# yahoo/bftkv

Hardware: AMD Instinct MI355X
Metric: pgp_rsa2048_signature_verifies_per_sec (higher is better)
Workload: dtype u32; 1 GPU; 64-replica quorum, 10000 RSA-2048 signed writes per GPU (cfg2 of BASELINE.json), 534164 signature packets per GPU, 1.0% corrupt / 0.5% unknown issuer / 0.5% duplicate / 1.0% one-short; parallelism=shard-by-write x1, RCCL all-gather of verdict bitmaps on the verifier's stream, replicas=64, writes_per_gpu=10000, sigs_per_gpu=534164, batches_in_flight=3

## Files before the change

### bftkv_amd/csrc/mont28.h

```cpp
#pragma once
#include <hip/hip_runtime.h>
#include <stdint.h>

namespace bftkv {

constexpr int MONT_W = 28;
constexpr uint32_t MONT_MASK = (1u << MONT_W) - 1;
constexpr int MONT_TPI = 4;
constexpr int MONT_L = 19;
constexpr int MONT_N = MONT_TPI * MONT_L;
constexpr int MONT_TPI_BIG = 8;
constexpr int MONT_L3072 = 14, MONT_L4096 = 19;
constexpr int MONT_NMAX = MONT_TPI_BIG * MONT_L4096;

constexpr int DPP_QUAD_BCAST0 = 0x00;
constexpr int DPP_QUAD_SHR1 = 0x90;
constexpr int DPP_QUAD_SWAP1 = 0xB1;
constexpr int DPP_QUAD_SWAP2 = 0x4E;
constexpr int DPP_ROW_SHL1 = 0x101;

__device__ __forceinline__ uint32_t dpp_quad_bcast0(uint32_t v) {
  return (uint32_t)__builtin_amdgcn_update_dpp(0, (int)v, DPP_QUAD_BCAST0, 0xF, 0xF, true);
}
__device__ __forceinline__ uint32_t dpp_quad_shr1(uint32_t v) {
  return (uint32_t)__builtin_amdgcn_update_dpp(0, (int)v, DPP_QUAD_SHR1, 0xF, 0xF, false);
}
__device__ __forceinline__ uint32_t dpp_row_shl1(uint32_t v) {
  return (uint32_t)__builtin_amdgcn_update_dpp(0, (int)v, DPP_ROW_SHL1, 0xF, 0xF, true);
}
constexpr int DPP_ROW_SHR1 = 0x111;
constexpr int DPP_ROW_SHR4 = 0x114;
__device__ __forceinline__ uint32_t dpp_row_shr1(uint32_t v) {
  return (uint32_t)__builtin_amdgcn_update_dpp(0, (int)v, DPP_ROW_SHR1, 0xF, 0xF, true);
}
__device__ __forceinline__ uint32_t dpp_row_shr4(uint32_t v) {
  return (uint32_t)__builtin_amdgcn_update_dpp(0, (int)v, DPP_ROW_SHR4, 0xF, 0xF, true);
}
__device__ __forceinline__ uint32_t quad_or(uint32_t v) {
  v |= (uint32_t)__builtin_amdgcn_update_dpp(0, (int)v, DPP_QUAD_SWAP1, 0xF, 0xF, false);
  v |= (uint32_t)__builtin_amdgcn_update_dpp(0, (int)v, DPP_QUAD_SWAP2, 0xF, 0xF, false);
  return v;
}

template <int TPI>
__device__ __forceinline__ uint32_t grp_bcast0(uint32_t v, int glane) {
  const uint32_t q = dpp_quad_bcast0(v);
  if constexpr (TPI == 4) return q;
  else { const uint32_t u = dpp_row_shr4(q); return (glane & 4) ? u : q; }
}
template <int TPI>
__device__ __forceinline__ uint32_t grp_shr1(uint32_t v) {
  if constexpr (TPI == 4) return dpp_quad_shr1(v);
  else return dpp_row_shr1(v);
}
template <int TPI>
__device__ __forceinline__ uint32_t grp_or(uint32_t v) {
  v = quad_or(v);
  if constexpr (TPI == 8) v |= (uint32_t)__shfl_xor((int)v, 4);
  return v;
}

__device__ __forceinline__ uint64_t mad64(uint32_t a, uint32_t b, uint64_t c) {
  return (uint64_t)a * (uint64_t)b + c;
}

template <int L, int TPI = MONT_TPI, bool SQR = false>
__device__ __forceinline__ void mont_mul(uint32_t (&out)[L], const uint32_t* a_lds,
                                         const uint32_t (&b)[L], const uint32_t (&n)[L],
                                         uint32_t n0inv, int qlane) {
  constexpr bool NORM = 2 * TPI * L > 255;
  uint32_t mask_v;
  asm("v_mov_b32 %0, 0xfffffff" : "=v"(mask_v));
  uint64_t Q[2 * L - 1];
#pragma unroll
  for (int k = 0; k < L + (NORM ? 1 : 0); ++k) Q[k] = 0;

#pragma unroll 1
  for (int blk = 0; blk < TPI; ++blk) {
    const uint32_t* ap = a_lds + blk * L;
#pragma unroll
    for (int r = 0; r < L; ++r) {
      const uint32_t ai = ap[r];
      const uint32_t ai2 = ai << 1;
#pragma unroll
      for (int k = SQR ? r : 0; k < L; ++k) {
        const uint32_t av = (SQR && k > r) ? ai2 : ai;
        if (k == L - 1 && r > 0) Q[r + k] = mad64(av, b[k], (NORM && r == 1) ? Q[r + k] : 0);
        else Q[r + k] = mad64(av, b[k], Q[r + k]);
      }
      const uint32_t m = grp_bcast0<TPI>((uint32_t)Q[r] * n0inv, qlane) & mask_v;
#pragma unroll
      for (int k = 0; k < L; ++k) Q[r + k] = mad64(m, n[k], Q[r + k]);
      Q[r + 1] += Q[r] >> MONT_W;
    }
#pragma unroll
    for (int k = 0; k < L; ++k) {
      const uint64_t nx = dpp_row_shl1((uint32_t)Q[k]) & mask_v;
      Q[k] = (k < L - 1) ? Q[L + k] + nx : nx;
    }
    if (NORM) {
#pragma unroll
      for (int k = 0; k < L; ++k) {
        const uint64_t c = Q[k] >> MONT_W;
        Q[k] &= MONT_MASK;
        if (k < L - 1) Q[k + 1] += c; else Q[L] = c;
      }
    }
  }

  uint64_t c = 0;
#pragma unroll
  for (int k = 0; k < L; ++k) {
    uint64_t v = Q[k] + c;
    out[k] = (uint32_t)v & MONT_MASK;
    c = v >> MONT_W;
  }
  if (NORM) c += Q[L];
  uint32_t clo = grp_shr1<TPI>((uint32_t)c), chi = grp_shr1<TPI>((uint32_t)(c >> 32));
  uint64_t cin = (qlane == 0) ? 0 : (((uint64_t)chi << 32) | clo);
  uint64_t v0 = (uint64_t)out[0] + cin;
  out[0] = (uint32_t)v0 & MONT_MASK;
  uint32_t v1 = out[1] + (uint32_t)(v0 >> MONT_W);
  out[1] = v1 & MONT_MASK;
  out[2] += v1 >> MONT_W;
}

template <int L, int TPI = MONT_TPI>
__device__ __forceinline__ void canonicalize(uint32_t (&x)[L], int qlane) {
  uint32_t cout = 0;
#pragma unroll
  for (int step = 0; step < TPI; ++step) {
    uint32_t c = grp_shr1<TPI>(cout);
    if (qlane == 0) c = 0;
#pragma unroll
    for (int k = 0; k < L; ++k) {
      uint32_t v = x[k] + c;
      x[k] = v & MONT_MASK;
      c = v >> MONT_W;
    }
    cout = c;
  }
}

template <int L, int TPI = MONT_TPI>
__device__ __forceinline__ void reduce_once(uint32_t (&y)[L], const uint32_t (&n)[L], int qlane) {
  uint32_t ge = 1;
#pragma unroll
  for (int k = 0; k < L; ++k) ge = (y[k] > n[k]) ? 1u : ((y[k] < n[k]) ? 0u : ge);
  if (!__any(ge != 0 && qlane == TPI - 1)) return;
  uint32_t d[L];
#pragma unroll
  for (int k = 0; k < L; ++k) d[k] = y[k] - n[k];
  int32_t cout = 0, top = 0;
#pragma unroll
  for (int step = 0; step < TPI; ++step) {
    int32_t c = (int32_t)grp_shr1<TPI>((uint32_t)cout);
    if (qlane == 0) c = 0;
#pragma unroll
    for (int k = 0; k < L; ++k) {
      const int32_t v = (int32_t)d[k] + c;
      d[k] = (uint32_t)v & MONT_MASK;
      c = v >> MONT_W;
    }
    cout = c;
    top += c;
  }
  uint32_t keep = (top == 0) ? 1u : 0u;
  if constexpr (TPI == 4) keep = (uint32_t)__builtin_amdgcn_update_dpp(0, (int)keep, 0xFF, 0xF, 0xF, true);
  else keep = (uint32_t)__shfl((int)keep, (int)((threadIdx.x & 63u) | (uint32_t)(TPI - 1)));
  if (keep) {
#pragma unroll
    for (int k = 0; k < L; ++k) y[k] = d[k];
  }
}

}
```

Baseline: 146.8 million verifies/s.

## Use a rotating ring window for the Montgomery accumulator instead of shifting Q

In the non-normalized path (RSA-2048: L=19, TPI=4), the accumulator Q becomes a 2L-entry ring with compile-time rotating offsets, and two limb-blocks are unrolled per loop iteration. This removes the per-block copy of Q[L+k] down to Q[k]. The cross-lane DPP shift-in is folded into the next row's final multiply-add instead of a separate pass. The cost is one extra 64-bit accumulator and a doubled unrolled body, which could raise VGPR pressure and code size.

```diff
diff --git a/bftkv_amd/csrc/mont28.h b/bftkv_amd/csrc/mont28.h
--- a/bftkv_amd/csrc/mont28.h
+++ b/bftkv_amd/csrc/mont28.h
@@ -64,41 +64,72 @@
   return (uint64_t)a * (uint64_t)b + c;
 }
 
+template <int L, int TPI, bool SQR, int O>
+__device__ __forceinline__ void mont_block_ring(uint64_t (&Q)[2 * L], const uint32_t* ap, const uint32_t (&b)[L],
+                                                const uint32_t (&n)[L], uint32_t n0inv, int qlane, uint32_t mask_v) {
+  constexpr int M = 2 * L;
+#pragma unroll
+  for (int r = 0; r < L; ++r) {
+    const uint32_t ai = ap[r];
+    const uint32_t ai2 = ai << 1;
+    uint64_t in = 0;
+    if (r > 0) in = dpp_row_shl1((uint32_t)Q[(O + r - 1) % M]) & mask_v;
+#pragma unroll
+    for (int k = SQR ? r : 0; k < L; ++k) {
+      const uint32_t av = (SQR && k > r) ? ai2 : ai;
+      if (k == L - 1 && r > 0) Q[(O + r + k) % M] = mad64(av, b[k], in);
+      else Q[(O + r + k) % M] = mad64(av, b[k], Q[(O + r + k) % M]);
+    }
+    const uint32_t m = grp_bcast0<TPI>((uint32_t)Q[(O + r) % M] * n0inv, qlane) & mask_v;
+#pragma unroll
+    for (int k = 0; k < L; ++k) Q[(O + r + k) % M] = mad64(m, n[k], Q[(O + r + k) % M]);
+    Q[(O + r + 1) % M] += Q[(O + r) % M] >> MONT_W;
+  }
+  Q[(O + M - 1) % M] = dpp_row_shl1((uint32_t)Q[(O + L - 1) % M]) & mask_v;
+}
+
 template <int L, int TPI = MONT_TPI, bool SQR = false>
 __device__ __forceinline__ void mont_mul(uint32_t (&out)[L], const uint32_t* a_lds,
                                          const uint32_t (&b)[L], const uint32_t (&n)[L],
                                          uint32_t n0inv, int qlane) {
   constexpr bool NORM = 2 * TPI * L > 255;
+  static_assert(TPI % 2 == 0, "the ring window runs two blocks per loop iteration");
   uint32_t mask_v;
   asm("v_mov_b32 %0, 0xfffffff" : "=v"(mask_v));
-  uint64_t Q[2 * L - 1];
+  uint64_t Q[NORM ? 2 * L - 1 : 2 * L];
 #pragma unroll
   for (int k = 0; k < L + (NORM ? 1 : 0); ++k) Q[k] = 0;
 
+  if constexpr (!NORM) {
 #pragma unroll 1
-  for (int blk = 0; blk < TPI; ++blk) {
-    const uint32_t* ap = a_lds + blk * L;
-#pragma unroll
-    for (int r = 0; r < L; ++r) {
-      const uint32_t ai = ap[r];
-      const uint32_t ai2 = ai << 1;
-#pragma unroll
-      for (int k = SQR ? r : 0; k < L; ++k) {
-        const uint32_t av = (SQR && k > r) ? ai2 : ai;
-        if (k == L - 1 && r > 0) Q[r + k] = mad64(av, b[k], (NORM && r == 1) ? Q[r + k] : 0);
-        else Q[r + k] = mad64(av, b[k], Q[r + k]);
+    for (int blk = 0; blk < TPI; blk += 2) {
+      mont_block_ring<L, TPI, SQR, 0>(Q, a_lds + blk * L, b, n, n0inv, qlane, mask_v);
+      mont_block_ring<L, TPI, SQR, L>(Q, a_lds + (blk + 1) * L, b, n, n0inv, qlane, mask_v);
+    }
+  } else {
+#pragma unroll 1
+    for (int blk = 0; blk < TPI; ++blk) {
+      const uint32_t* ap = a_lds + blk * L;
+#pragma unroll
+      for (int r = 0; r < L; ++r) {
+        const uint32_t ai = ap[r];
+        const uint32_t ai2 = ai << 1;
+#pragma unroll
+        for (int k = SQR ? r : 0; k < L; ++k) {
+          const uint32_t av = (SQR && k > r) ? ai2 : ai;
+          if (k == L - 1 && r > 0) Q[r + k] = mad64(av, b[k], (r == 1) ? Q[r + k] : 0);
+          else Q[r + k] = mad64(av, b[k], Q[r + k]);
+        }
+        const uint32_t m = grp_bcast0<TPI>((uint32_t)Q[r] * n0inv, qlane) & mask_v;
+#pragma unroll
+        for (int k = 0; k < L; ++k) Q[r + k] = mad64(m, n[k], Q[r + k]);
+        Q[r + 1] += Q[r] >> MONT_W;
       }
-      const uint32_t m = grp_bcast0<TPI>((uint32_t)Q[r] * n0inv, qlane) & mask_v;
-#pragma unroll
-      for (int k = 0; k < L; ++k) Q[r + k] = mad64(m, n[k], Q[r + k]);
-      Q[r + 1] += Q[r] >> MONT_W;
-    }
-#pragma unroll
-    for (int k = 0; k < L; ++k) {
-      const uint64_t nx = dpp_row_shl1((uint32_t)Q[k]) & mask_v;
-      Q[k] = (k < L - 1) ? Q[L + k] + nx : nx;
-    }
-    if (NORM) {
+#pragma unroll
+      for (int k = 0; k < L; ++k) {
+        const uint64_t nx = dpp_row_shl1((uint32_t)Q[k]) & mask_v;
+        Q[k] = (k < L - 1) ? Q[L + k] + nx : nx;
+      }
 #pragma unroll
       for (int k = 0; k < L; ++k) {
         const uint64_t c = Q[k] >> MONT_W;
```

Result: faster. 153.0 million verifies/s, median of 6 (+4.2%).
